# indianajohn/akaze-rust

Hardware: AMD Instinct MI355X
Metric: Mpix/s through extract_features (4 oct x 4 sub) (higher is better)
Workload: dtype f32

## Files before the change

### akaze-rust_amd/csrc/akz_api.cpp

```cpp
#include "akz_ctx.hpp"

unsigned akz::host_cpu_share() {
    unsigned n = std::max(1u, std::thread::hardware_concurrency());
    cpu_set_t set;
    if (sched_getaffinity(0, sizeof(set), &set) == 0) n = std::max(1, CPU_COUNT(&set));
    if (FILE* f = fopen("/sys/fs/cgroup/cpu.max", "r")) {
        char q[32] = {0};
        long period = 0;
        if (fscanf(f, "%31s %ld", q, &period) == 2 && period > 0 && strcmp(q, "max") != 0)
            n = std::min<unsigned>(n, (unsigned)std::max(1L, atol(q) / period));
        fclose(f);
    }
    if (const char* e = std::getenv("LOCAL_WORLD_SIZE")) {
        const int ranks = atoi(e);
        if (ranks > 1) n = std::max(2u, n / (unsigned)ranks);
    }
    return std::max(1u, n);
}

int level_info_out(const std::vector<LevelPlan>& plan, uint64_t level, double* etime, double* esigma,
                          uint32_t* octave, uint32_t* sublevel, uint32_t* sigma_size, uint32_t* lw, uint32_t* lh,
                          uint32_t* det_sigma, uint64_t* n_tau, double* tau, uint64_t tau_cap) {
    if (level >= plan.size()) {
        set_error("level out of range");
// ... 375 lines not shown
    for (int k = 0; k < akz_ctx::kSlots; ++k)
        if (c->slot_busy[k]) {
            set_error("akz_ctx_set_host_threads: extractions are in flight on this context");
            return AKZ_ERR_INVALID_ARG;
        }
    c->host_threads = threads;
    c->workers.reset();
    for (akz_ctx* l : c->lanes) AKZ_TRY(akz_ctx_set_host_threads(l, threads));
    return AKZ_OK;
}
int akz_ctx_set_candidate_hint(akz_ctx* c, uint32_t per_image) {
    AKZ_TRY(bind(c));
    c->cand_cap_hint = std::max<uint32_t>(per_image, 16u);
    for (akz_ctx* l : c->lanes) l->cand_cap_hint = c->cand_cap_hint.load();
    return AKZ_OK;
}
int akz_ctx_set_match_mode(akz_ctx* c, int mode) {
    AKZ_TRY(bind(c));
    if (mode < 0 || mode > 3) return AKZ_ERR_INVALID_ARG;
    c->match_mode = mode;
    for (akz_ctx* l : c->lanes) l->match_mode = mode;
    return AKZ_OK;
}
int akz_ctx_set_fed_mode(akz_ctx* c, int mode) {
    AKZ_TRY(bind(c));
    if (mode != 0 && mode != 2) return AKZ_ERR_INVALID_ARG;
    c->fed_mode = mode;
    for (akz_ctx* l : c->lanes) l->fed_mode = mode;
    return AKZ_OK;
}
const char* akz_fed_kernel_name(void) { return "k_level_march + k_fed_own"; }
int akz_debug_march_bands(int kind, uint32_t w, uint32_t h, uint32_t n, int half_width, int32_t* rows, uint32_t cap,
                          uint32_t* n_bands) {
    if (!n_bands || (cap && !rows) || kind < 0 || kind > 1 || w < 16 || h < 16 || n == 0 || half_width < 1 || half_width > 4)
        return AKZ_ERR_INVALID_ARG;
    *n_bands = launch::march_band_rows(kind, w, h, n, half_width, rows, cap);
    return AKZ_OK;
}
const char* akz_detector_kernel_name(void) { return "detector (k_detector_march + k_detector_tiled)"; }
int akz_debug_set_schedule(akz_ctx* c, int key, int value) {
    if (!c || key < 0 || key > 10) return AKZ_ERR_INVALID_ARG;
    AKZ_TRY(bind(c));
    c->sched[key] = value;
    if (key == 7 || key == 8) launch::march_min_band_rows(c->sched[7], c->sched[8]);
    if (key == 4) {
        c->big_px_sync = value > 0 ? (uint64_t)value * 1000u : gates::kBigPxSync;
        c->big_px_async = value > 0 ? (uint64_t)value * 1000u : gates::kBigPxAsync;
        c->lane_px = value > 0 ? (uint64_t)value * 1000u : gates::kLanePx;
        for (akz_ctx* l : c->lanes) {
            l->big_px_sync = std::max(c->big_px_sync, c->lane_px);
            l->big_px_async = std::max(c->big_px_async, c->lane_px);
        }
    }
    return AKZ_OK;
}
int akz_debug_placement_verdict(float spin_pair_ms, float tiny_pair_ms, float tiny_alone_ms, float spin_ms) {
    return akz::placement_verdict(spin_pair_ms, tiny_pair_ms, tiny_alone_ms, spin_ms);
}
int akz_debug_stream_placement(akz_ctx* c, int* info) {
    if (!c || !info) return AKZ_ERR_INVALID_ARG;
    AKZ_TRY(bind(c));
    info[0] = c->placed ? 1 : 0;
    info[1] = c->pre_mode;
    info[2] = c->place_replaced;
    info[3] = c->place_collisions + c->lane_collisions;
    return AKZ_OK;
}
int akz_debug_select_info(akz_ctx* c, int* info) {
    if (!c || !info) return AKZ_ERR_INVALID_ARG;
    AKZ_TRY(bind(c));
    const akz_ctx* q = c->lanes.empty() ? c : c->lanes[0];
    info[0] = q->sel_last_mode.load();
    info[1] = (int)q->sel_last_rounds.load();
    info[2] = (int)q->sel_last_fallback.load();
    info[3] = (int)q->last_total_cands.load();
    for (int k = 0; k < 4; ++k) info[4 + k] = (int)q->sel_last_ticks[k].load();
    return AKZ_OK;
// ... 76 lines not shown
```

### akaze-rust_amd/csrc/akz_ctx.hpp

```cpp
#pragma once
#include <algorithm>
#include <cmath>
#include <cstdlib>
#include <cstddef>
#include <cstring>
#include <atomic>
#include <condition_variable>
#include <functional>
#include <map>
#include <memory>
#include <mutex>
#include <thread>
#include <sched.h>
#include <time.h>
#include <type_traits>

#include "akz_internal.hpp"
#include "akz_select.hpp"
#include "akz_pool.hpp"
#include "akz_gates.hpp"

#define AKZ_LOCAL __attribute__((visibility("hidden")))

namespace akz {
// ... 92 lines not shown
    int dbg_device_libm = -1;
    int libm_last = 0;
    int dbg_host_sort = -1;
    DevBuf cosi;
    DevBuf pin[PIN_COUNT_];
    std::vector<std::pair<size_t, void*>> slab_pool;
    std::mutex slab_m;
    static constexpr int kSlots = 3;
    DevBuf cand_slot[kSlots], count_slot[kSlots];
    std::atomic<bool> slot_busy[kSlots] = {{false}, {false}, {false}};
    std::atomic<uint32_t> cand_cap_hint{1u << 15};
    std::atomic<int> live_results{0};
    bool dead = false;
    std::atomic<uint32_t> last_total_cands{0};
    std::atomic<uint64_t> last_cand_shape{0};
    hipStream_t aux = nullptr;
    std::mutex aux_m;
    hipStream_t coarse = nullptr;
    hipStream_t pre = nullptr;
    hipEvent_t pre_done = nullptr;
    hipStream_t copy = nullptr;
    DevBuf stage[kSlots];
    hipEvent_t staged[kSlots] = {nullptr, nullptr, nullptr};
    std::vector<akz_ctx*> lanes;
    unsigned next_lane = 0;
    bool is_lane = false;
    bool eager_finish = true;
    std::shared_ptr<Finisher> fin;
    hipEvent_t lane_in = nullptr;
    uint64_t stream_min_px = gates::kStreamPx;
    int prep_mode = 2;
    int det_mode = 2;
    int fed_mode = 2;
    int sched[11] = {0, 1, 0, 0, 0, 0, 0, 0, 0, 0, 0};
    uint64_t big_px = gates::kBigPxAsync;
    uint64_t big_px_sync = gates::kBigPxSync, big_px_async = gates::kBigPxAsync;
    uint64_t lane_px = gates::kLanePx;
    static constexpr uint64_t kLaunchMarchPx = gates::kMarchPx;
    uint64_t launch_min_px = kLaunchMarchPx;
    bool placed = false;
    int pre_mode = 0;
    int place_replaced = 0;
    int place_collisions = 0;
    int place_retries = 0;
    int lane_collisions = 0;
    hipEvent_t probe_ev[2] = {nullptr, nullptr};
    int profiling = 0;
    akz_profile prof{};
    struct Span { int stage; hipEvent_t a, b; int row; };
    std::vector<Span> spans;
    std::vector<akz_kernel_row> rows;
    std::vector<hipEvent_t> ev_pool;
    std::mutex ev_m;
    static constexpr int kFedRing = 4;
    hipEvent_t fed_ev[kFedRing] = {nullptr, nullptr, nullptr, nullptr};
    hipEvent_t pre_ev[kFedRing] = {nullptr, nullptr, nullptr, nullptr};
    std::atomic<uint64_t> begin_seq{0};
    std::shared_ptr<std::atomic<int>> in_hand = std::make_shared<std::atomic<int>>(0);
    std::unique_ptr<WorkerPool> workers;
    unsigned host_threads = 0;
    WorkerPool& pool() {
        if (!workers) workers.reset(new WorkerPool(std::min(host_threads ? host_threads : host_cpu_share(), 16u) - 1));
        return *workers;
    }
    hipStream_t fetch[2] = {nullptr, nullptr};
    DevBuf fetch_stage;
    hipEvent_t fetch_chunk[4] = {nullptr, nullptr, nullptr, nullptr};
// ... 221 lines not shown
```

### akaze-rust_amd/csrc/akz_extract_begin.cpp

```cpp
#include "akz_extract.hpp"

namespace {
enum class Prep : uint8_t {
    Tiled,
    Stream,
    LevelMarch,
    Resident
};
enum class Det : uint8_t {
    Fallback,
    NmsFused,
    TiledSet,
    March
};
struct BeginRoute {
    bool big = false;
    int prep_mode = 0;
    int pre_on = 0;
    bool level1_clone = false;
    size_t res_first = 0;
    size_t fork_level = 0;
    size_t oct1 = 0;
    bool own_kernels = true;
    struct Level {
// ... 31 lines not shown
            if (plan[l].tau.empty()) ok = false;
            steps += plan[l].tau.size();
            if (steps > (size_t)launch::kResidentMaxSteps) {
                steps -= plan[l].tau.size();
                f = l + 1;
                break;
            }
        }
        if (ok && f < L) rt.res_first = f;
    }
    rt.fork_level = L;
    if (fork_octave > 0 && c->profiling < 2 && big)
        for (size_t i = 1; i < L && rt.fork_level == L; ++i)
            if ((int)plan[i].octave >= fork_octave) rt.fork_level = i;
    if (rt.fork_level < L && rt.res_first < rt.fork_level) rt.fork_level = rt.res_first;
    rt.oct1 = 1;
    while (rt.oct1 < rt.fork_level && plan[rt.oct1].octave == plan[0].octave) ++rt.oct1;

    for (size_t l = 0; l < L; ++l) {
        const LevelPlan& lv = plan[l];
        BeginRoute::Level& q = rt.lv[l];
        const int fam = detector_family(c, lv.det_sigma, lv.w, lv.h, n, border_margin(lv, cfg), (flags & AKZ_KEEP_ALL_PLANES) != 0);
        q.det = fam == 5 ? Det::March : fam == 4 ? Det::TiledSet : launch::detector_nms_fused_supported(lv.det_sigma) ? Det::NmsFused : Det::Fallback;
        if (l >= rt.fork_level && q.det == Det::Fallback) rt.own_kernels = false;
        if (l == 0) continue;
        const LevelPlan& pv = plan[l - 1];
        const bool half = lv.octave > pv.octave;
        const uint64_t lpx = (uint64_t)lv.w * lv.h * n;
        if (l >= rt.res_first) {
            q.prep = Prep::Resident;
        } else if (!lv.tau.empty() && c->fed_mode == 2 && launch::level_march_supported(lv.w, lv.h) &&
                   (c->prep_mode == 3 || (c->prep_mode == 2 && lpx >= gates::kLevelMarchPx))) {
            q.prep = Prep::LevelMarch;
            q.n1 = std::min<uint32_t>((uint32_t)lv.tau.size(), 4u);
            q.rem = (uint32_t)lv.tau.size() - q.n1;
            q.fold_half = half && launch::level_march_half_supported(lv.w, lv.h, pv.w, pv.h, q.n1);
        } else if (c->prep_mode != 0 && launch::prep_stream_supported(lv.w, lv.h) &&
                   (c->prep_mode == 1 || (c->prep_mode >= 2 && !half && lpx >= c->stream_min_px))) {
            q.prep = Prep::Stream;
        }
        q.may_ride = c->sched[6] == 0 && c->fed_mode == 2 && lv.octave == pv.octave && q.prep == Prep::Tiled;
    }
    return rt;
}

struct BeginState {
    akz_ctx* c;
    akz_result* r;
    const BeginRoute& rt;
    uint32_t n;
    bool keep_all;
    hipStream_t s;
    hipStream_t ls;
    uint64_t seq;
    Candidate* d_cand;
    uint32_t* d_count;
    uint32_t cap;
    std::vector<float> g1;
    std::vector<char> det_done;
    std::vector<char> prepared;
    bool head_fused = false;
    float* P(size_t l, int p) const { return r->planes[l][p]; }
    size_t L() const { return r->plan.size(); }
};

bool detector_one_pass(BeginState& b, size_t l, hipStream_t on) {
    akz_ctx* c = b.c;
// ... 64 lines not shown
    for (size_t l = i; l < L; ++l) {
        for (double t : plan[l].tau) ht[l].push_back(0.5f * (float)t);
        rl.push_back(launch::ResidentLevel{b.P(l, AKZ_LT), b.P(l, AKZ_LSMOOTH), b.P(l, AKZ_LFLOW), b.keep_all ? b.P(l, AKZ_LSTEP) : nullptr,
                                           plan[l].w, plan[l].h, plan[l].octave > plan[l - 1].octave,
                                           (uint32_t)plan[l].tau.size(), ht[l].data(), plan[l].octave});
        px_steps += (uint64_t)plan[l].w * plan[l].h * b.n * plan[l].tau.size();
    }
    StageTimer st(c, AKZ_ST_FED);
    st.kernel(AKZ_KR_OCTAVE_RESIDENT, (uint32_t)rl.size(), plan[i].w, plan[i].h, b.n, 1, 0, px_steps);
    launch::octave_resident(b.ls, b.P(i - 1, AKZ_LT), plan[i - 1].w, plan[i - 1].h, b.n, rl.data(), (uint32_t)rl.size(), b.g1.data(), b.r->d_k);
    if (c->profiling) {
        c->prof.fed_launches += 1;
        c->prof.fed_px_steps += px_steps;
    }
    AKZ_HIP_TRY(hipGetLastError());
    return AKZ_OK;
}

int level_by_march(BeginState& b, size_t i, float* A, float* B) {
    akz_ctx* c = b.c;
    const LevelPlan &lv = b.r->plan[i], &pv = b.r->plan[i - 1];
    const BeginRoute::Level& q = b.rt.lv[i];
    const uint32_t n = b.n, n1 = q.n1, rem = q.rem;
    const bool half = lv.octave > pv.octave;
    const uint32_t rest = rem ? fed_num_launches(c, rem, lv.w, lv.h, n) : 0;
    float* d1 = fed_dst(rest + 1, 1, A, B);
    const float* level_in = b.P(i - 1, AKZ_LT);
    if (half && !q.fold_half) {
        StageTimer st(c, AKZ_ST_PREP);
        float* hb = d1 == A ? B : A;
        launch::half_size(b.ls, b.P(i - 1, AKZ_LT), hb, pv.w, pv.h, n);
        level_in = hb;
    }
    float ht[4];
    for (uint32_t j = 0; j < n1; ++j) ht[j] = 0.5f * (float)lv.tau[j];
    {
        StageTimer st(c, AKZ_ST_FED);
        st.kernel(AKZ_KR_LEVEL_MARCH, n1 | (q.fold_half ? 16u : 0u) | ((rem == 0 && b.keep_all) ? 32u : 0u), lv.w, lv.h, n, 1,
                  (uint64_t)lv.w * lv.h * n, (uint64_t)lv.w * lv.h * n * n1);
        launch::level_march(b.ls, level_in, b.P(i, AKZ_LSMOOTH), b.P(i, AKZ_LFLOW), d1,
                            (rem == 0 && b.keep_all) ? b.P(i, AKZ_LSTEP) : nullptr, lv.w, lv.h, n, b.g1.data(), b.r->d_k,
                            lv.octave, ht, n1, q.fold_half ? pv.w : 0u, q.fold_half ? pv.h : 0u);
        if (c->profiling) {
            c->prof.fed_launches += 1;
            c->prof.fed_px_steps += (uint64_t)lv.w * lv.h * n * n1;
            c->prof.fused_px += (uint64_t)lv.w * lv.h * n;
        }
    }
    if (rem) {
        StageTimer st(c, AKZ_ST_FED);
        st.kernel(AKZ_KR_FED_OWN, rem, lv.w, lv.h, n, rest, 0, (uint64_t)lv.w * lv.h * n * rem);
        AKZ_TRY(fed_impl(c, d1, A, B, b.P(i, AKZ_LFLOW), b.keep_all ? b.P(i, AKZ_LSTEP) : nullptr, lv.w, lv.h, n, lv.tau.data() + n1, rem));
    }
    AKZ_HIP_TRY(hipGetLastError());
    return AKZ_OK;
}

int level_by_launches(BeginState& b, size_t i, float* A, float* B) {
    akz_ctx* c = b.c;
    const LevelPlan &lv = b.r->plan[i], &pv = b.r->plan[i - 1];
    const uint32_t n = b.n, n_tau = (uint32_t)lv.tau.size();
    const bool half = lv.octave > pv.octave;
    const float* fed_in = b.P(i - 1, AKZ_LT);
    float* half_buf = nullptr;
    if (half) {
        const uint32_t launches = fed_num_launches(c, n_tau, lv.w, lv.h, n);
        half_buf = launches == 0 ? A : (fed_dst(launches, 1, A, B) == A ? B : A);
// ... 203 lines not shown
```

### akaze-rust_amd/csrc/akz_internal.hpp

```cpp
#pragma once
#include <hip/hip_runtime.h>

#include <cstdint>
#include <functional>
#include <string>
#include <vector>

#include "../../include/akaze_hip.h"
#include "../../include/akaze_hip_debug.h"

namespace akz {

void set_error(const std::string& msg);
unsigned host_cpu_share();

using TrialsOnDevice = std::function<int(const float*, const float*, const float*, const float*, uint32_t, const uint32_t*, uint32_t,
                                         float, float, float*, int32_t*)>;
int remove_outliers_impl(const akz_keypoint* keypoints_0, uint64_t n0, const akz_keypoint* keypoints_1, uint64_t n1,
                         const akz_match* matches, uint64_t n_matches, uint64_t num_trials, float epsilon_model,
                         float epsilon_inlier, akz_match* out, uint64_t* n_out, const TrialsOnDevice& trials_on_device);

#define AKZ_HIP_TRY(expr)                                                                          \
    do {                                                                                           \
        hipError_t _e = (expr);                                                                    \
// ... 148 lines not shown
                          float thr, float border_m, Candidate* d_cand, uint32_t cap, uint32_t* d_count);
bool blur5_stream_supported(uint32_t w, uint32_t h, uint32_t ntaps, bool is_u8);
void blur5_stream_u8(hipStream_t s, const uint8_t* in, float* out, uint32_t w, uint32_t h, uint32_t n, const float* k);
void blur5_stream_f32(hipStream_t s, const float* in, float* out, uint32_t w, uint32_t h, uint32_t n, const float* k);
uint32_t march_band_rows(int kind, uint32_t w, uint32_t h, uint32_t n, int S, int32_t* cs_ce, uint32_t cap);
bool blur5_march_supported(uint32_t w, uint32_t h, uint32_t ntaps);
void blur5_march_u8(hipStream_t s, const uint8_t* in, float* out, uint32_t w, uint32_t h, uint32_t n, const float* k);
void blur5_march_f32(hipStream_t s, const float* in, float* out, uint32_t w, uint32_t h, uint32_t n, const float* k);
bool contrast_march_supported(uint32_t w, uint32_t h, uint32_t ntaps, uint32_t nbins);
void contrast_march(hipStream_t s, const float* in, uint32_t w, uint32_t h, uint32_t n, const float* g3,
                    unsigned long long* d_hmax_bits, uint32_t nbins, uint32_t* d_hist, double* d_thr);
void contrast_thresholds(hipStream_t s, const unsigned long long* d_hmax_bits, uint32_t nbins, uint32_t n, double* d_thr);
bool contrast_stream_supported(uint32_t w, uint32_t h, uint32_t ntaps, uint32_t nbins);
void contrast_stream(hipStream_t s, const float* in, uint32_t w, uint32_t h, uint32_t n, const float* g3,
                     unsigned long long* d_hmax_bits, uint32_t nbins, uint32_t* d_hist, double* d_thr);
bool prep_stream_supported(uint32_t w, uint32_t h);
void prep_stream(hipStream_t s, const float* prev, bool half, float* lt_out, float* lsmooth, float* lflow, uint32_t w,
                 uint32_t h, uint32_t pw, uint32_t ph, uint32_t n, const float* g3, const double* d_k, uint32_t k_pow);
bool detector_march_supported(uint32_t sigma, uint32_t w, uint32_t h, float border_m, bool nms);
void detector_march(hipStream_t s, const float* lsmooth, uint32_t sigma, float* lx, float* ly, float* lxx, float* lyy,
                    float* lxy, float* ldet_out, uint32_t w, uint32_t h, uint32_t n, uint32_t level, float thr,
                    float border_m, Candidate* d_cand, uint32_t cap, uint32_t* d_count);
bool head_fused_supported(uint32_t w, uint32_t h, uint32_t ntaps0, uint32_t ntaps1);
void head_fused_u8(hipStream_t s, const uint8_t* in, float* lt0, float* blurred, float* gx, float* gy, uint32_t w, uint32_t h, uint32_t n,
                   const float* k5, const float* g3, unsigned long long* d_smax_bits, uint32_t* d_zero_word = nullptr);
void head_fused_f32(hipStream_t s, const float* in, float* lt0, float* blurred, float* gx, float* gy, uint32_t w, uint32_t h, uint32_t n,
                    const float* k5, const float* g3, unsigned long long* d_smax_bits, uint32_t* d_zero_word = nullptr);
void contrast_hist_final(hipStream_t s, const float* gx, const float* gy, uint32_t w, uint32_t h, uint32_t n, unsigned long long* d_smax_bits,
                         uint32_t nbins, uint32_t* d_hist, uint32_t* d_done, double percentile, double* d_k);
void flow_from_pair(hipStream_t s, const float* gx, const float* gy, float* lflow, uint32_t w, uint32_t h, uint32_t n, const double* d_k,
                    uint32_t k_pow);
void march_min_band_rows(int detector, int level);
bool level_march_supported(uint32_t w, uint32_t h);
bool level_march_half_supported(uint32_t w, uint32_t h, uint32_t pw, uint32_t ph, uint32_t n_steps);
void level_march(hipStream_t s, const float* prev, float* lsmooth, float* lflow, float* lt_out, float* lstep, uint32_t w,
                 uint32_t h, uint32_t n, const float* g3, const double* d_k, uint32_t k_pow, const float* half_taus,
                 uint32_t n_steps, uint32_t pw = 0, uint32_t ph = 0);
struct ResidentLevel {
    float *lt, *lsmooth, *lflow, *lstep;
    uint32_t w, h;
    bool half;
    uint32_t n_tau;
    const float* half_tau;
    uint32_t k_pow;
};
constexpr int kResidentMaxLevels = 10;
constexpr int kResidentMaxSteps = 448;
bool octave_resident_supported(uint32_t w, uint32_t h);
void octave_resident(hipStream_t s, const float* prev, uint32_t pw, uint32_t ph, uint32_t n, const ResidentLevel* levels,
                     uint32_t n_levels, const float* g3, const double* d_k);
bool detector_nms_fused_supported(uint32_t sigma);
void detector_nms_fused(hipStream_t s, const float* lsmooth, uint32_t sigma, float* lx, float* ly, float* lxx,
                        float* lyy, float* lxy, float* ldet_out, uint32_t w, uint32_t h, uint32_t n, uint32_t level,
                        float thr, float border_m, Candidate* d_cand, uint32_t cap, uint32_t* d_count);
void rcp_f64_to_f32(hipStream_t s, const double* x, float* out, uint64_t n);
void accumulate(hipStream_t s, float* a, const float* b, uint64_t count);
void ldet(hipStream_t s, const float* lxx, const float* lyy, const float* lxy, float* out, uint64_t count,
          float sigma_quat);
size_t sort_candidates_scratch(uint32_t cap, uint64_t max_px, uint32_t n_levels, uint32_t n_images);
uint32_t sort_small_capacity();
size_t sort_candidates_buckets_scratch(uint32_t cap);
bool sort_candidates_buckets(hipStream_t s, const Candidate* d_cand, uint32_t cap, const uint32_t* d_count, const uint32_t* level_w,
                             const uint32_t* level_h, uint32_t n_levels, uint32_t n_images, void* scratch, bool scratch_is_new,
                             Candidate* d_sorted, uint32_t* d_zero, void* rel_scratch);
bool sort_candidates_rows(hipStream_t s, const Candidate* d_cand, uint32_t cap, const uint32_t* d_count, const uint32_t* level_w,
                          const uint32_t* level_h, uint32_t n_levels, Candidate* d_sorted, uint32_t* d_zero, void* rel_scratch);
// ... 128 lines not shown
```

### akaze-rust_amd/csrc/akz_march.hip

```cpp
#include <hip/hip_runtime.h>

#include <algorithm>
#include <cstdlib>
#include <type_traits>

#include "akz_internal.hpp"
#include "akz_pm_g2.hpp"

namespace akz {
namespace {

typedef float f2 __attribute__((ext_vector_type(2)));
typedef float f2u __attribute__((ext_vector_type(2), aligned(4)));

constexpr int MT = 256;
constexpr int MW = 2 * MT;
constexpr int HALO = 16;
constexpr int USE = MW - 2 * HALO;
constexpr int PAD = 8;
constexpr int ROW = MW + 2 * PAD;
constexpr int CBUF = 32;
#ifndef AKZ_MARCH_PF
#define AKZ_MARCH_PF 3
#endif
// ... 293 lines not shown
                if (NMS) {
                    const int y = c - 1;
                    if (y >= cs && y < ce && y >= nms.ylo && y <= nms.yhi) {
                        const float* dr = buf + 3 * ROW + wi;
                        const float left = dr[-1], right = dr[2];
                        const bool h0 = (dm1.x > nms.thr) & (dm1.x > dm1.y) & (dm1.x > left) & (dm1.x > dm2.x) & (dm1.x > det.x);
                        const bool h1 = (dm1.y > nms.thr) & (dm1.y > right) & (dm1.y > dm1.x) & (dm1.y > dm2.y) & (dm1.y > det.y);
                        const unsigned m = ((h0 ? 1u : 0u) | (h1 ? 2u : 0u)) & xok;
                        cands_push(cbuf, cnum, m, nms, lane, [&](int i) {
                            Candidate cd;
                            cd.level = nms.level;
                            cd.idx = (unsigned)(y * w + C.x0 + i);
                            cd.v = i == 0 ? dm1.x : dm1.y;
                            cd.xp = i == 0 ? dm1.y : right;
                            cd.xm = i == 0 ? left : dm1.x;
                            cd.yp = i == 0 ? det.x : det.y;
                            cd.ym = i == 0 ? dm2.x : dm2.y;
                            cd.img = (unsigned)img;
                            return cd;
                        });
                    }
                    dm2 = dm1;
                    dm1 = det;
                }
                lx_c = lx_n;
                ly_c = ly_n;
            }
        }
    }
    if (NMS) cands_flush(cbuf, cnum, nms, lane);
}

struct LevelTaus {
    float half_tau[4];
};
__device__ __forceinline__ f2 lds2(const float* p) { return f2{p[0], p[1]}; }
__device__ __forceinline__ f2 tap3(f2 a, f2 b, f2 c, float k0, float k1, float k2) {
    const f2 z = {0.0f, 0.0f};
    return ((z + k0 * a) + k1 * b) + k2 * c;
}
__device__ __forceinline__ double octave_contrast(double k, unsigned pow) {
    for (unsigned i = 0; i < pow; ++i) k = k * 0.75;
    return k;
}

typedef unsigned u4m __attribute__((ext_vector_type(4)));
template <int N, bool KEEPSTEP, bool ODDW, bool HALF = false>
__global__ void __launch_bounds__(MT, 3)
k_level_march(const float* __restrict__ prev, float* __restrict__ lsmooth_out, float* __restrict__ lflow_out,
              float* __restrict__ lt_out, float* __restrict__ lstep_out, int w, int h, MarchGrid g, float g0, float g1,
              float g2, float kn, float kwn, const double* __restrict__ d_k, unsigned k_pow, LevelTaus ht, int pw = 0, int ph = 0) {
    static_assert(!(HALF && ODDW), "the 2x2 mean is folded in for even level widths only");
    static_assert(N >= 1 && N <= 4, "fused diffusion steps");
    static_assert(N + 3 <= HALO, "strip halo");
    constexpr int NPL = 3 + N;
#ifndef AKZ_LEVEL_PF
#define AKZ_LEVEL_PF 2
#endif
    constexpr int PF = AKZ_LEVEL_PF;
    static_assert(PF >= 1 && PF <= 3, "prefetch ring");
    __shared__ __attribute__((aligned(16))) float s_row[2][NPL][ROW];
    const int tid = threadIdx.x;
    const int per = g.nbands * g.nstrips;
    const int cell = march_cell();
    if (cell >= g.total) return;
    const int img = __builtin_amdgcn_readfirstlane(cell / per);
    const int rem = cell - img * per;
    const int band = __builtin_amdgcn_readfirstlane(rem / g.nstrips), strip = rem - band * g.nstrips;
    int cs, ce;
    level_band_rows(g, band, h, &cs, &ce);
    if (cs >= ce) return;
    const int lt0 = cs == 1 ? 0 : cs, lt1 = ce == h - 1 ? h : ce;

    const int X0 = strip * USE - HALO;
    const int p0 = (2 * tid + HALO) & (MW - 1);
    const bool inner = p0 >= HALO && p0 < MW - HALO;
    const Cols C = make_cols(X0 + p0, inner, w);
    const int i0 = PAD + clampi(clampi(C.x0, 1, w - 2) - X0, 0, MW - 1) - 1;
    const int i1 = PAD + clampi(clampi(C.x0 + 1, 1, w - 2) - X0, 0, MW - 1) - 1;
    const int wi = PAD + p0;
    const bool edge_h = __ballot(i0 != wi - 1 || i1 != wi) != 0ull;
    const bool hxn0 = C.x0 > 0, hxp0 = C.x0 + 1 < w, hxn1 = C.x0 + 1 > 0, hxp1 = C.x0 + 2 < w;
    const bool edge_col = __ballot(!(hxn0 && hxp0 && hxn1 && hxp1)) != 0ull;

    const size_t base = (size_t)img * (size_t)w * (size_t)h;
    const __amdgpu_buffer_rsrc_t in = HALF ? plane_rsrc(prev + (size_t)img * (size_t)pw * (size_t)ph, pw, ph) : plane_rsrc(prev + base, w, h);
    const __amdgpu_buffer_rsrc_t o_ls[1] = {plane_rsrc(lsmooth_out + base, w, h)};
    const __amdgpu_buffer_rsrc_t o_lf[1] = {plane_rsrc(lflow_out + base, w, h)};
    __amdgpu_buffer_rsrc_t o_lt[KEEPSTEP ? 2 : 1];
    o_lt[0] = plane_rsrc(lt_out + base, w, h);
    if (KEEPSTEP) o_lt[1] = plane_rsrc(lstep_out + base, w, h);
    const __amdgpu_buffer_rsrc_t(&o_ltc)[KEEPSTEP ? 2 : 1] = o_lt;
    const double kc = octave_contrast(d_k[img], k_pow);
    const double inverse_k = 1.0 / (kc * kc);

    const int v0 = lt0 - N - 2;
    const int T = (lt1 - lt0) + 2 * N + 6;
    struct Fed {
        f2 v;
        u4m top, bot;
    };
    auto feed = [&](int t) -> Fed {
        Fed f;
        const unsigned row = (unsigned)clampi(v0 + min(t, T - 1), 0, h - 1);
        if constexpr (HALF) {
            const unsigned ro = 2u * row * ((unsigned)pw * 4u);
            f.top = __builtin_amdgcn_raw_buffer_load_b128(in, (int)(2u * C.vo_ld), (int)ro, 0);
            f.bot = __builtin_amdgcn_raw_buffer_load_b128(in, (int)(2u * C.vo_ld), (int)(ro + (unsigned)pw * 4u), 0);
        } else {
            f.v = load_pair<ODDW>(in, row * ((unsigned)w * 4u), C);
        }
        return f;
    };
    auto pair_of = [&](const Fed& f) -> f2 {
        if constexpr (HALF) {
            float a = 0.0f, b = 0.0f;
            a = a + __uint_as_float(f.top.x); a = a + __uint_as_float(f.bot.x); a = a + __uint_as_float(f.top.y); a = a + __uint_as_float(f.bot.y);
            b = b + __uint_as_float(f.top.z); b = b + __uint_as_float(f.bot.z); b = b + __uint_as_float(f.top.w); b = b + __uint_as_float(f.bot.w);
            return f2{a / 4.0f, b / 4.0f};
        } else {
            return f.v;
        }
    };
    Fed q[4];
#pragma unroll
    for (int i = 0; i < PF; ++i) q[i] = feed(i);
    const f2 zero = {0.0f, 0.0f};
    f2 LP[8], CR[8];
    f2 GH[4], HM[4], HO[4];
    f2 SXW[4], SXE[4];
    f2 W[N > 1 ? N - 1 : 1][4];
#pragma unroll
    for (int i = 0; i < 8; ++i) LP[i] = CR[i] = zero;
#pragma unroll
    for (int i = 0; i < 4; ++i) {
        GH[i] = HM[i] = HO[i] = SXW[i] = SXE[i] = zero;
#pragma unroll
        for (int j = 0; j < (N > 1 ? N - 1 : 1); ++j) W[j][i] = zero;
    }
    f2 ls_c = zero, lf_c = zero, gh_c = zero;

    auto rows = [&](auto mid_tag) {
    constexpr bool MID = decltype(mid_tag)::value;
    for (int t0 = 0; t0 < T; t0 += 8) {
#pragma unroll
        for (int k = 0; k < 8; ++k) {
            const int t = t0 + k;
            {
                const int v = v0 + t;
                q[(k + PF) & 3] = feed(t + PF);
                float* const buf = &s_row[t & 1][0][0];
                LP[k & 7] = fix_pair(pair_of(q[k & 3]), C);
                *reinterpret_cast<f2*>(buf + 0 * ROW + wi) = LP[k & 7];
                *reinterpret_cast<f2*>(buf + 1 * ROW + wi) = ls_c;
                *reinterpret_cast<f2*>(buf + 2 * ROW + wi) = CR[(k - 5) & 7];
                *reinterpret_cast<f2*>(buf + 3 * ROW + wi) = LP[(k - 5) & 7];
#pragma unroll
                for (int s = 2; s <= N; ++s) *reinterpret_cast<f2*>(buf + (2 + s) * ROW + wi) = W[s - 2][(k - 1) & 3];
                __syncthreads();
                f2 gh = gh_c;
                if (MID || v <= h - 2) {
                    f2 a, b, c;
                    if (!rare(edge_h)) {
                        a = lds2(buf + wi - 1); b = LP[k & 7]; c = lds2(buf + wi + 1);
                    } else {
                        const float* r0 = buf + i0;
                        const float* r1 = buf + i1;
                        a = f2{r0[0], r1[0]}; b = f2{r0[1], r1[1]}; c = f2{r0[2], r1[2]};
                    }
                    gh = tap3(a, b, c, g0, g1, g2);
                }
                gh_c = gh;
                GH[k & 3] = gh;
                if (!MID && rare(v == 1)) GH[(k - 1) & 3] = gh;
                const int u = v - 1;
                f2 ls_n = ls_c;
                if (MID || u <= h - 2) ls_n = tap3(GH[(k - 2) & 3], GH[(k - 1) & 3], GH[k & 3], g0, g1, g2);
                {
                    const f2 o[1] = {ls_n};
                    if (MID) store_rows<1, ODDW>(o_ls, u, w, u >= cs && u < ce, C, o);
                    else store_filled<1, 1, ODDW>(o_ls, C, w, h, u, u >= cs && u < ce, o);
                }
                {
                    f2 a, b, c;
                    if (!rare(edge_h)) {
                        a = lds2(buf + ROW + wi - 1); b = ls_c; c = lds2(buf + ROW + wi + 1);
                    } else {
                        const float* r0 = buf + ROW + i0;
                        const float* r1 = buf + ROW + i1;
                        a = f2{r0[0], r1[0]}; b = f2{r0[1], r1[1]}; c = f2{r0[2], r1[2]};
                    }
                    HM[k & 3] = tap_main(a, b, c, kn, kwn);
                    HO[k & 3] = tap_off(a, c);
                }
                if (!MID && rare(u - 1 == 1)) {
                    HM[(k - 1) & 3] = HM[k & 3];
                    HO[(k - 1) & 3] = HO[k & 3];
                }
                const int c = v - 3;
                f2 lf_n = lf_c;
                if (MID || c <= h - 2) {
                    const f2 lx1 = tap_off(HM[(k - 2) & 3], HM[k & 3]);
                    const f2 ly1 = tap_main(HO[(k - 2) & 3], HO[(k - 1) & 3], HO[k & 3], kn, kwn);
                    lf_n = f2{pm_g2_px(lx1.x, ly1.x, inverse_k), pm_g2_px(lx1.y, ly1.y, inverse_k)};
                }
                CR[(k - 3) & 7] = lf_n;
                if (!MID && rare(c == 1)) CR[(k - 4) & 7] = lf_n;
                {
                    const f2 o[1] = {lf_n};
                    if (MID) store_rows<1, ODDW>(o_lf, c, w, c >= cs && c < ce, C, o);
                    else store_filled<1, 1, ODDW>(o_lf, C, w, h, c, c >= cs && c < ce, o);
                }
                {
                    const float* cr = buf + 2 * ROW + wi;
                    const f2 cc = CR[(k - 5) & 7];
                    SXW[k & 3] = lds2(cr - 1) + cc;
                    SXE[k & 3] = cc + lds2(cr + 1);
                }
                f2 lnew = zero, st = zero;
#pragma unroll
                for (int s = 1; s <= N; ++s) {
                    const int r = v - 4 - s;
                    f2 Lm, Lc, Lp;
                    if (s == 1) {
                        Lm = LP[(k - 6) & 7]; Lc = LP[(k - 5) & 7]; Lp = LP[(k - 4) & 7];
                    } else {
                        W[s - 2][k & 3] = lnew;
                        Lm = W[s - 2][(k - 2) & 3]; Lc = W[s - 2][(k - 1) & 3]; Lp = lnew;
                    }
                    const float* lr = buf + (2 + s) * ROW + wi;
                    const f2 Lw = lds2(lr - 1), Le = lds2(lr + 1);
                    const f2 cN = CR[(k - 5 - s) & 7], cC = CR[(k - 4 - s) & 7], cS = CR[(k - 3 - s) & 7];
                    const f2 SU = cN + cC, SV = cC + cS;
                    const f2 XFW = SXW[(k - (s - 1)) & 3] * (Lc - Lw);
                    const f2 XFE = SXE[(k - (s - 1)) & 3] * (Le - Lc);
                    f2 tx;
                    if (!edge_col) {
                        tx = XFE - XFW;
                    } else {
                        tx.x = hxp0 ? (hxn0 ? XFE.x - XFW.x : XFE.x) : -XFW.x;
                        tx.y = hxp1 ? (hxn1 ? XFE.y - XFW.y : XFE.y) : -XFW.y;
                    }
                    f2 tt;
                    if (MID || r + 1 < h) {
                        tt = tx + SV * (Lp - Lc);
                        if (MID || r > 0) tt = tt - SU * (Lc - Lm);
                    } else {
                        tt = tx + SU * (Lm - Lc);
                    }
                    st = ht.half_tau[s - 1] * tt;
                    lnew = Lc + st;
                }
                {
                    const int r = v - 4 - N;
                    {
                        f2 o[KEEPSTEP ? 2 : 1];
                        o[0] = lnew;
                        if constexpr (KEEPSTEP) o[1] = st;
                        const f2(&oc)[KEEPSTEP ? 2 : 1] = o;
                        store_rows<KEEPSTEP ? 2 : 1, ODDW>(o_ltc, r, w, r >= lt0 && r < lt1, C, oc);
                    }
                }
                ls_c = ls_n;
                lf_c = lf_n;
            }
        }
    }
    };
    const int v_last = v0 + ((T + 7) & ~7) - 1;
    if (v0 >= N + 5 && v_last <= h - 2) rows(std::true_type{});
    else rows(std::false_type{});
// ... 416 lines not shown
    else hipLaunchKernelGGL((k_blur5_march<T, false>), gr, dim3(MT), 0, s, in, out, (int)w, (int)h, mg, tp);
}
void blur5_march_u8(hipStream_t s, const uint8_t* in, float* out, uint32_t w, uint32_t h, uint32_t n, const float* k) {
    blur5_march_t<uint8_t>(s, in, out, w, h, n, k);
}
void blur5_march_f32(hipStream_t s, const float* in, float* out, uint32_t w, uint32_t h, uint32_t n, const float* k) {
    blur5_march_t<float>(s, in, out, w, h, n, k);
}

bool contrast_march_supported(uint32_t w, uint32_t h, uint32_t ntaps, uint32_t nbins) {
    return ntaps == 3 && nbins >= 1 && nbins <= 640 && level_march_supported(w, h);
}
void contrast_march(hipStream_t s, const float* in, uint32_t w, uint32_t h, uint32_t n, const float* g3,
                    unsigned long long* d_hmax_bits, uint32_t nbins, uint32_t* d_hist, double* d_thr) {
    const Taps m = taps_scharr_main(1);
    const ContrastMarchArgs ca{d_hmax_bits, d_hist, nbins, d_thr};
    dim3 gr;
    const MarchGrid mg = plan_level_march(w, h, n, &gr, 8, g_head_min_rows > 0 ? g_head_min_rows : 32);
    if (w & 1u)
        hipLaunchKernelGGL((k_contrast_march<1, true>), gr, dim3(MT), 0, s, in, (int)w, (int)h, mg, g3[0], g3[1], g3[2], m.wgt[0], m.wgt[1], ca);
    else
        hipLaunchKernelGGL((k_contrast_march<1, false>), gr, dim3(MT), 0, s, in, (int)w, (int)h, mg, g3[0], g3[1], g3[2], m.wgt[0], m.wgt[1], ca);
    contrast_thresholds(s, d_hmax_bits, nbins, n, d_thr);
    const size_t lds = ((size_t)(MT / 64) * CM_COPIES * nbins) * sizeof(unsigned) + (size_t)(nbins + 1) * sizeof(double);
    if (w & 1u)
        hipLaunchKernelGGL((k_contrast_march<2, true>), gr, dim3(MT), lds, s, in, (int)w, (int)h, mg, g3[0], g3[1], g3[2], m.wgt[0], m.wgt[1], ca);
    else
        hipLaunchKernelGGL((k_contrast_march<2, false>), gr, dim3(MT), lds, s, in, (int)w, (int)h, mg, g3[0], g3[1], g3[2], m.wgt[0], m.wgt[1], ca);
}

#ifndef AKZ_LVL_FILL
#define AKZ_LVL_FILL 3
#endif
static int level_min_band_rows(uint32_t w, uint32_t h, uint32_t n) {
    if (g_lvl_min_rows > 0) return g_lvl_min_rows;
    return (uint64_t)w * h * n < (48u << 20) ? 20 : 64;
}
uint32_t march_band_rows(int kind, uint32_t w, uint32_t h, uint32_t n, int S, int32_t* cs_ce, uint32_t cap) {
    dim3 gr;
    const MarchGrid g = kind == 1 ? plan_level_march(w, h, n, &gr, AKZ_LVL_FILL, level_min_band_rows(w, h, n)) : plan_march(w, h, n, S, &gr);
    for (int b = 0; b < g.nbands && (uint32_t)b < cap; ++b) {
        int cs, ce;
        if (kind == 1) level_band_rows(g, b, (int)h, &cs, &ce);
        else uniform_band_rows(g, b, S, (int)h, &cs, &ce);
        cs_ce[2 * b] = cs;
        cs_ce[2 * b + 1] = ce;
    }
    return (uint32_t)g.nbands;
}

bool level_march_supported(uint32_t w, uint32_t h) { return w >= 16 && h >= 16 && (uint64_t)w * h <= (1ull << 28); }

template <int NS, bool KEEPSTEP>
static void launch_level_march(hipStream_t s, dim3 gr, const MarchGrid& mg, const float* prev, float* lsmooth, float* lflow,
                               float* lt_out, float* lstep, uint32_t w, uint32_t h, const float* g3, const Taps& m,
                               const double* d_k, uint32_t k_pow, const LevelTaus& ht, uint32_t pw, uint32_t ph) {
    if constexpr (NS == 4) {
        if (pw) {
            hipLaunchKernelGGL((k_level_march<NS, KEEPSTEP, false, true>), gr, dim3(MT), 0, s, prev, lsmooth, lflow, lt_out, lstep, (int)w,
                               (int)h, mg, g3[0], g3[1], g3[2], m.wgt[0], m.wgt[1], d_k, k_pow, ht, (int)pw, (int)ph);
            return;
        }
    }
    if (w & 1u)
        hipLaunchKernelGGL((k_level_march<NS, KEEPSTEP, true>), gr, dim3(MT), 0, s, prev, lsmooth, lflow, lt_out, lstep, (int)w,
                           (int)h, mg, g3[0], g3[1], g3[2], m.wgt[0], m.wgt[1], d_k, k_pow, ht);
    else
        hipLaunchKernelGGL((k_level_march<NS, KEEPSTEP, false>), gr, dim3(MT), 0, s, prev, lsmooth, lflow, lt_out, lstep, (int)w,
                           (int)h, mg, g3[0], g3[1], g3[2], m.wgt[0], m.wgt[1], d_k, k_pow, ht);
}
#define AKZ_LEVEL(NS)                                                                                                        \
    case NS: {                                                                                                               \
        if (lstep) launch_level_march<NS, true>(s, gr, mg, prev, lsmooth, lflow, lt_out, lstep, w, h, g3, m, d_k, k_pow, ht, pw, ph);  \
        else launch_level_march<NS, false>(s, gr, mg, prev, lsmooth, lflow, lt_out, lstep, w, h, g3, m, d_k, k_pow, ht, pw, ph);       \
    } break;

bool level_march_half_supported(uint32_t w, uint32_t h, uint32_t pw, uint32_t ph, uint32_t n_steps) {
    return n_steps == 4 && (pw & 3u) == 0 && (w & 1u) == 0 && w == pw / 2 && h == ph / 2 && (uint64_t)pw * ph <= (1ull << 28);
}
void level_march(hipStream_t s, const float* prev, float* lsmooth, float* lflow, float* lt_out, float* lstep, uint32_t w,
                 uint32_t h, uint32_t n, const float* g3, const double* d_k, uint32_t k_pow, const float* half_taus,
                 uint32_t n_steps, uint32_t pw, uint32_t ph) {
    const Taps m = taps_scharr_main(1);
    LevelTaus ht;
    for (uint32_t i = 0; i < 4; ++i) ht.half_tau[i] = i < n_steps ? half_taus[i] : 0.0f;
    dim3 gr;
    const MarchGrid mg = plan_level_march(w, h, n, &gr, AKZ_LVL_FILL, level_min_band_rows(w, h, n));
    switch (n_steps) {
        AKZ_LEVEL(1) AKZ_LEVEL(2) AKZ_LEVEL(3) AKZ_LEVEL(4)
        default: break;
    }
}
#undef AKZ_LEVEL

}
}
```

Measured before the change: 15030.

## Fuse up to seven FED diffusion steps into one level-march kernel

The level-march kernel now accepts 5 to 7 fused explicit diffusion steps for even-width levels that are not the first of an octave. It uses LDS-backed previous rows and a shorter register window, plus extra conductivity history registers. This avoids a separate remainder pass over the level when the FED cycle has more than four steps. The cost is a deeper halo, larger minimum band rows, more registers and LDS per block, and recomputed edge-column handling. A schedule knob can restore the four-step cap.

```diff
diff --git a/akaze-rust_amd/csrc/akz_api.cpp b/akaze-rust_amd/csrc/akz_api.cpp
--- a/akaze-rust_amd/csrc/akz_api.cpp
+++ b/akaze-rust_amd/csrc/akz_api.cpp
@@ -431,17 +431,19 @@
 const char* akz_fed_kernel_name(void) { return "k_level_march + k_fed_own"; }
 int akz_debug_march_bands(int kind, uint32_t w, uint32_t h, uint32_t n, int half_width, int32_t* rows, uint32_t cap,
                           uint32_t* n_bands) {
-    if (!n_bands || (cap && !rows) || kind < 0 || kind > 1 || w < 16 || h < 16 || n == 0 || half_width < 1 || half_width > 4)
+    if (!n_bands || (cap && !rows) || kind < 0 || kind > 2 || w < 16 || h < 16 || n == 0 || half_width < 1 || half_width > (kind == 2 ? 7 : 4))
         return AKZ_ERR_INVALID_ARG;
     *n_bands = launch::march_band_rows(kind, w, h, n, half_width, rows, cap);
     return AKZ_OK;
 }
 const char* akz_detector_kernel_name(void) { return "detector (k_detector_march + k_detector_tiled)"; }
 int akz_debug_set_schedule(akz_ctx* c, int key, int value) {
-    if (!c || key < 0 || key > 10) return AKZ_ERR_INVALID_ARG;
+    if (!c || key < 0 || key > 11) return AKZ_ERR_INVALID_ARG;
     AKZ_TRY(bind(c));
     c->sched[key] = value;
     if (key == 7 || key == 8) launch::march_min_band_rows(c->sched[7], c->sched[8]);
+    if (key == 11)
+        for (akz_ctx* l : c->lanes) l->sched[11] = value;
     if (key == 4) {
         c->big_px_sync = value > 0 ? (uint64_t)value * 1000u : gates::kBigPxSync;
         c->big_px_async = value > 0 ? (uint64_t)value * 1000u : gates::kBigPxAsync;
diff --git a/akaze-rust_amd/csrc/akz_ctx.hpp b/akaze-rust_amd/csrc/akz_ctx.hpp
--- a/akaze-rust_amd/csrc/akz_ctx.hpp
+++ b/akaze-rust_amd/csrc/akz_ctx.hpp
@@ -148,7 +148,7 @@
     int prep_mode = 2;
     int det_mode = 2;
     int fed_mode = 2;
-    int sched[11] = {0, 1, 0, 0, 0, 0, 0, 0, 0, 0, 0};
+    int sched[12] = {0, 1, 0, 0, 0, 0, 0, 0, 0, 0, 0, 0};
     uint64_t big_px = gates::kBigPxAsync;
     uint64_t big_px_sync = gates::kBigPxSync, big_px_async = gates::kBigPxAsync;
     uint64_t lane_px = gates::kLanePx;
diff --git a/akaze-rust_amd/csrc/akz_extract_begin.cpp b/akaze-rust_amd/csrc/akz_extract_begin.cpp
--- a/akaze-rust_amd/csrc/akz_extract_begin.cpp
+++ b/akaze-rust_amd/csrc/akz_extract_begin.cpp
@@ -87,7 +87,9 @@
         } else if (!lv.tau.empty() && c->fed_mode == 2 && launch::level_march_supported(lv.w, lv.h) &&
                    (c->prep_mode == 3 || (c->prep_mode == 2 && lpx >= gates::kLevelMarchPx))) {
             q.prep = Prep::LevelMarch;
-            q.n1 = std::min<uint32_t>((uint32_t)lv.tau.size(), 4u);
+            const uint32_t n_tau = (uint32_t)lv.tau.size();
+            const uint32_t cap = c->sched[11] ? 4u : launch::level_march_max_steps(lv.w, lv.h, half);
+            q.n1 = n_tau <= cap ? n_tau : std::min<uint32_t>(n_tau, 4u);
             q.rem = (uint32_t)lv.tau.size() - q.n1;
             q.fold_half = half && launch::level_march_half_supported(lv.w, lv.h, pv.w, pv.h, q.n1);
         } else if (c->prep_mode != 0 && launch::prep_stream_supported(lv.w, lv.h) &&
@@ -218,7 +220,7 @@
         launch::half_size(b.ls, b.P(i - 1, AKZ_LT), hb, pv.w, pv.h, n);
         level_in = hb;
     }
-    float ht[4];
+    float ht[7];
     for (uint32_t j = 0; j < n1; ++j) ht[j] = 0.5f * (float)lv.tau[j];
     {
         StageTimer st(c, AKZ_ST_FED);
diff --git a/akaze-rust_amd/csrc/akz_internal.hpp b/akaze-rust_amd/csrc/akz_internal.hpp
--- a/akaze-rust_amd/csrc/akz_internal.hpp
+++ b/akaze-rust_amd/csrc/akz_internal.hpp
@@ -204,6 +204,7 @@
                     uint32_t k_pow);
 void march_min_band_rows(int detector, int level);
 bool level_march_supported(uint32_t w, uint32_t h);
+uint32_t level_march_max_steps(uint32_t w, uint32_t h, bool half);
 bool level_march_half_supported(uint32_t w, uint32_t h, uint32_t pw, uint32_t ph, uint32_t n_steps);
 void level_march(hipStream_t s, const float* prev, float* lsmooth, float* lflow, float* lt_out, float* lstep, uint32_t w,
                  uint32_t h, uint32_t n, const float* g3, const double* d_k, uint32_t k_pow, const float* half_taus,
diff --git a/akaze-rust_amd/csrc/akz_march.hip b/akaze-rust_amd/csrc/akz_march.hip
--- a/akaze-rust_amd/csrc/akz_march.hip
+++ b/akaze-rust_amd/csrc/akz_march.hip
@@ -349,7 +349,7 @@
 }
 
 struct LevelTaus {
-    float half_tau[4];
+    float half_tau[7];
 };
 __device__ __forceinline__ f2 lds2(const float* p) { return f2{p[0], p[1]}; }
 __device__ __forceinline__ f2 tap3(f2 a, f2 b, f2 c, float k0, float k1, float k2) {
@@ -368,9 +368,14 @@
               float* __restrict__ lt_out, float* __restrict__ lstep_out, int w, int h, MarchGrid g, float g0, float g1,
               float g2, float kn, float kwn, const double* __restrict__ d_k, unsigned k_pow, LevelTaus ht, int pw = 0, int ph = 0) {
     static_assert(!(HALF && ODDW), "the 2x2 mean is folded in for even level widths only");
-    static_assert(N >= 1 && N <= 4, "fused diffusion steps");
+    static_assert(N >= 1 && N <= 7, "fused diffusion steps");
+    static_assert(N <= 4 || !(ODDW || HALF), "more than four fused steps: even widths, not the first level of an octave");
     static_assert(N + 3 <= HALO, "strip halo");
     constexpr int NPL = 3 + N;
+    constexpr bool DEEP = N > 4;
+    constexpr int CXN = N > 5 ? N - 5 : 0;
+    constexpr int SXN = DEEP ? 8 : 4;
+    constexpr int WN = DEEP ? 1 : 4;
 #ifndef AKZ_LEVEL_PF
 #define AKZ_LEVEL_PF 2
 #endif
@@ -397,6 +402,13 @@
     const int i1 = PAD + clampi(clampi(C.x0 + 1, 1, w - 2) - X0, 0, MW - 1) - 1;
     const int wi = PAD + p0;
     const bool edge_h = __ballot(i0 != wi - 1 || i1 != wi) != 0ull;
+    auto col_here = [&]() -> int {
+        int x = C.x0;
+        asm volatile("" : "+v"(x));
+        return x;
+    };
+    auto tap_i0 = [&](int x) -> int { return PAD + clampi(clampi(x, 1, w - 2) - X0, 0, MW - 1) - 1; };
+    auto tap_i1 = [&](int x) -> int { return PAD + clampi(clampi(x + 1, 1, w - 2) - X0, 0, MW - 1) - 1; };
     const bool hxn0 = C.x0 > 0, hxp0 = C.x0 + 1 < w, hxn1 = C.x0 + 1 > 0, hxp1 = C.x0 + 2 < w;
     const bool edge_col = __ballot(!(hxn0 && hxp0 && hxn1 && hxp1)) != 0ull;
 
@@ -445,15 +457,25 @@
     const f2 zero = {0.0f, 0.0f};
     f2 LP[8], CR[8];
     f2 GH[4], HM[4], HO[4];
-    f2 SXW[4], SXE[4];
-    f2 W[N > 1 ? N - 1 : 1][4];
+    f2 SXW[SXN], SXE[SXN];
+    f2 W[N > 1 ? N - 1 : 1][WN];
+    f2 CX[CXN > 0 ? CXN : 1];
 #pragma unroll
     for (int i = 0; i < 8; ++i) LP[i] = CR[i] = zero;
 #pragma unroll
-    for (int i = 0; i < 4; ++i) {
-        GH[i] = HM[i] = HO[i] = SXW[i] = SXE[i] = zero;
+    for (int i = 0; i < (CXN > 0 ? CXN : 1); ++i) CX[i] = zero;
+#pragma unroll
+    for (int i = 0; i < SXN; ++i) SXW[i] = SXE[i] = zero;
+#pragma unroll
+    for (int i = 0; i < 4; ++i) GH[i] = HM[i] = HO[i] = zero;
+#pragma unroll
+    for (int i = 0; i < WN; ++i) {
 #pragma unroll
         for (int j = 0; j < (N > 1 ? N - 1 : 1); ++j) W[j][i] = zero;
+    }
+    if constexpr (DEEP) {
+#pragma unroll
+        for (int s = 1; s <= N; ++s) *reinterpret_cast<f2*>(&s_row[1][2 + s][wi]) = zero;
     }
     f2 ls_c = zero, lf_c = zero, gh_c = zero;
 
@@ -467,13 +489,23 @@
                 const int v = v0 + t;
                 q[(k + PF) & 3] = feed(t + PF);
                 float* const buf = &s_row[t & 1][0][0];
-                LP[k & 7] = fix_pair(pair_of(q[k & 3]), C);
+                if constexpr (DEEP) {
+                    f2 lp = pair_of(q[k & 3]);
+                    if (rare(C.ld_edge)) {
+                        const int x = col_here();
+                        if (x < 0) lp.y = lp.x;
+                        if (x > w - 2) lp.x = lp.y;
+                    }
+                    LP[k & 7] = lp;
+                } else {
+                    LP[k & 7] = fix_pair(pair_of(q[k & 3]), C);
+                }
                 *reinterpret_cast<f2*>(buf + 0 * ROW + wi) = LP[k & 7];
                 *reinterpret_cast<f2*>(buf + 1 * ROW + wi) = ls_c;
                 *reinterpret_cast<f2*>(buf + 2 * ROW + wi) = CR[(k - 5) & 7];
                 *reinterpret_cast<f2*>(buf + 3 * ROW + wi) = LP[(k - 5) & 7];
 #pragma unroll
-                for (int s = 2; s <= N; ++s) *reinterpret_cast<f2*>(buf + (2 + s) * ROW + wi) = W[s - 2][(k - 1) & 3];
+                for (int s = 2; s <= N; ++s) *reinterpret_cast<f2*>(buf + (2 + s) * ROW + wi) = W[s - 2][(k - 1) & (WN - 1)];
                 __syncthreads();
                 f2 gh = gh_c;
                 if (MID || v <= h - 2) {
@@ -481,8 +513,9 @@
                     if (!rare(edge_h)) {
                         a = lds2(buf + wi - 1); b = LP[k & 7]; c = lds2(buf + wi + 1);
                     } else {
-                        const float* r0 = buf + i0;
-                        const float* r1 = buf + i1;
+                        const int x = DEEP ? col_here() : 0;
+                        const float* r0 = buf + (DEEP ? tap_i0(x) : i0);
+                        const float* r1 = buf + (DEEP ? tap_i1(x) : i1);
                         a = f2{r0[0], r1[0]}; b = f2{r0[1], r1[1]}; c = f2{r0[2], r1[2]};
                     }
                     gh = tap3(a, b, c, g0, g1, g2);
@@ -503,8 +536,9 @@
                     if (!rare(edge_h)) {
                         a = lds2(buf + ROW + wi - 1); b = ls_c; c = lds2(buf + ROW + wi + 1);
                     } else {
-                        const float* r0 = buf + ROW + i0;
-                        const float* r1 = buf + ROW + i1;
+                        const int x = DEEP ? col_here() : 0;
+                        const float* r0 = buf + ROW + (DEEP ? tap_i0(x) : i0);
+                        const float* r1 = buf + ROW + (DEEP ? tap_i1(x) : i1);
                         a = f2{r0[0], r1[0]}; b = f2{r0[1], r1[1]}; c = f2{r0[2], r1[2]};
                     }
                     HM[k & 3] = tap_main(a, b, c, kn, kwn);
@@ -521,6 +555,10 @@
                     const f2 ly1 = tap_main(HO[(k - 2) & 3], HO[(k - 1) & 3], HO[k & 3], kn, kwn);
                     lf_n = f2{pm_g2_px(lx1.x, ly1.x, inverse_k), pm_g2_px(lx1.y, ly1.y, inverse_k)};
                 }
+                if constexpr (CXN > 0) {
+                    if constexpr (CXN > 1) CX[1] = CX[0];
+                    CX[0] = CR[(k - 3) & 7];
+                }
                 CR[(k - 3) & 7] = lf_n;
                 if (!MID && rare(c == 1)) CR[(k - 4) & 7] = lf_n;
                 {
@@ -531,8 +569,8 @@
                 {
                     const float* cr = buf + 2 * ROW + wi;
                     const f2 cc = CR[(k - 5) & 7];
-                    SXW[k & 3] = lds2(cr - 1) + cc;
-                    SXE[k & 3] = cc + lds2(cr + 1);
+                    SXW[k & (SXN - 1)] = lds2(cr - 1) + cc;
+                    SXE[k & (SXN - 1)] = cc + lds2(cr + 1);
                 }
                 f2 lnew = zero, st = zero;
 #pragma unroll
@@ -540,20 +578,36 @@
                     const int r = v - 4 - s;
                     f2 Lm, Lc, Lp;
                     if (s == 1) {
-                        Lm = LP[(k - 6) & 7]; Lc = LP[(k - 5) & 7]; Lp = LP[(k - 4) & 7];
+                        if constexpr (DEEP) Lm = *reinterpret_cast<const f2*>(&s_row[(t - 1) & 1][3][wi]);
+                        else Lm = LP[(k - 6) & 7];
+                        Lc = LP[(k - 5) & 7]; Lp = LP[(k - 4) & 7];
+                    } else if constexpr (DEEP) {
+                        Lm = *reinterpret_cast<const f2*>(&s_row[(t - 1) & 1][2 + s][wi]);
+                        Lc = W[s - 2][0]; Lp = lnew;
+                        W[s - 2][0] = lnew;
                     } else {
                         W[s - 2][k & 3] = lnew;
                         Lm = W[s - 2][(k - 2) & 3]; Lc = W[s - 2][(k - 1) & 3]; Lp = lnew;
                     }
                     const float* lr = buf + (2 + s) * ROW + wi;
                     const f2 Lw = lds2(lr - 1), Le = lds2(lr + 1);
-                    const f2 cN = CR[(k - 5 - s) & 7], cC = CR[(k - 4 - s) & 7], cS = CR[(k - 3 - s) & 7];
+                    auto c_row = [&](int m) -> f2 {
+                        if constexpr (CXN > 0) {
+                            if (m > 10) return CX[m - 11];
+                        }
+                        return CR[(k - m) & 7];
+                    };
+                    const f2 cN = c_row(5 + s), cC = c_row(4 + s), cS = c_row(3 + s);
                     const f2 SU = cN + cC, SV = cC + cS;
-                    const f2 XFW = SXW[(k - (s - 1)) & 3] * (Lc - Lw);
-                    const f2 XFE = SXE[(k - (s - 1)) & 3] * (Le - Lc);
+                    const f2 XFW = SXW[(k - (s - 1)) & (SXN - 1)] * (Lc - Lw);
+                    const f2 XFE = SXE[(k - (s - 1)) & (SXN - 1)] * (Le - Lc);
                     f2 tx;
                     if (!edge_col) {
                         tx = XFE - XFW;
+                    } else if constexpr (DEEP) {
+                        const int x = col_here();
+                        tx.x = x + 1 < w ? (x > 0 ? XFE.x - XFW.x : XFE.x) : -XFW.x;
+                        tx.y = x + 2 < w ? (x + 1 > 0 ? XFE.y - XFW.y : XFE.y) : -XFW.y;
                     } else {
                         tx.x = hxp0 ? (hxn0 ? XFE.x - XFW.x : XFE.x) : -XFW.x;
                         tx.y = hxp1 ? (hxn1 ? XFE.y - XFW.y : XFE.y) : -XFW.y;
@@ -1036,16 +1090,18 @@
 #ifndef AKZ_LVL_FILL
 #define AKZ_LVL_FILL 3
 #endif
-static int level_min_band_rows(uint32_t w, uint32_t h, uint32_t n) {
+static int level_min_band_rows(uint32_t w, uint32_t h, uint32_t n, uint32_t n_steps = 4) {
     if (g_lvl_min_rows > 0) return g_lvl_min_rows;
-    return (uint64_t)w * h * n < (48u << 20) ? 20 : 64;
+    const int rows = (uint64_t)w * h * n < (48u << 20) ? 20 : 64;
+    return n_steps > 4 ? std::max(rows, 2 * (2 * (int)n_steps + 6)) : rows;
 }
 uint32_t march_band_rows(int kind, uint32_t w, uint32_t h, uint32_t n, int S, int32_t* cs_ce, uint32_t cap) {
     dim3 gr;
-    const MarchGrid g = kind == 1 ? plan_level_march(w, h, n, &gr, AKZ_LVL_FILL, level_min_band_rows(w, h, n)) : plan_march(w, h, n, S, &gr);
+    const MarchGrid g = kind >= 1 ? plan_level_march(w, h, n, &gr, AKZ_LVL_FILL, level_min_band_rows(w, h, n, kind == 2 ? (uint32_t)S : 4u))
+                                  : plan_march(w, h, n, S, &gr);
     for (int b = 0; b < g.nbands && (uint32_t)b < cap; ++b) {
         int cs, ce;
-        if (kind == 1) level_band_rows(g, b, (int)h, &cs, &ce);
+        if (kind >= 1) level_band_rows(g, b, (int)h, &cs, &ce);
         else uniform_band_rows(g, b, S, (int)h, &cs, &ce);
         cs_ce[2 * b] = cs;
         cs_ce[2 * b + 1] = ce;
@@ -1066,7 +1122,11 @@
             return;
         }
     }
-    if (w & 1u)
+    if constexpr (NS > 4) {
+        hipLaunchKernelGGL((k_level_march<NS, KEEPSTEP, false>), gr, dim3(MT), 0, s, prev, lsmooth, lflow, lt_out, lstep, (int)w,
+                           (int)h, mg, g3[0], g3[1], g3[2], m.wgt[0], m.wgt[1], d_k, k_pow, ht);
+        return;
+    } else if (w & 1u)
         hipLaunchKernelGGL((k_level_march<NS, KEEPSTEP, true>), gr, dim3(MT), 0, s, prev, lsmooth, lflow, lt_out, lstep, (int)w,
                            (int)h, mg, g3[0], g3[1], g3[2], m.wgt[0], m.wgt[1], d_k, k_pow, ht);
     else
@@ -1079,6 +1139,10 @@
         else launch_level_march<NS, false>(s, gr, mg, prev, lsmooth, lflow, lt_out, lstep, w, h, g3, m, d_k, k_pow, ht, pw, ph);       \
     } break;
 
+uint32_t level_march_max_steps(uint32_t w, uint32_t h, bool half) {
+    (void)h;
+    return (half || (w & 1u)) ? 4u : 7u;
+}
 bool level_march_half_supported(uint32_t w, uint32_t h, uint32_t pw, uint32_t ph, uint32_t n_steps) {
     return n_steps == 4 && (pw & 3u) == 0 && (w & 1u) == 0 && w == pw / 2 && h == ph / 2 && (uint64_t)pw * ph <= (1ull << 28);
 }
@@ -1087,11 +1151,11 @@
                  uint32_t n_steps, uint32_t pw, uint32_t ph) {
     const Taps m = taps_scharr_main(1);
     LevelTaus ht;
-    for (uint32_t i = 0; i < 4; ++i) ht.half_tau[i] = i < n_steps ? half_taus[i] : 0.0f;
+    for (uint32_t i = 0; i < 7; ++i) ht.half_tau[i] = i < n_steps ? half_taus[i] : 0.0f;
     dim3 gr;
-    const MarchGrid mg = plan_level_march(w, h, n, &gr, AKZ_LVL_FILL, level_min_band_rows(w, h, n));
+    const MarchGrid mg = plan_level_march(w, h, n, &gr, AKZ_LVL_FILL, level_min_band_rows(w, h, n, n_steps));
     switch (n_steps) {
-        AKZ_LEVEL(1) AKZ_LEVEL(2) AKZ_LEVEL(3) AKZ_LEVEL(4)
+        AKZ_LEVEL(1) AKZ_LEVEL(2) AKZ_LEVEL(3) AKZ_LEVEL(4) AKZ_LEVEL(5) AKZ_LEVEL(6) AKZ_LEVEL(7)
         default: break;
     }
 }
```

Result: no change. 15180, median of 6 (+1.0%).
